# Cyan4973/FiniteStateEntropy

Measured on NVIDIA H100. Metric: encode+decode GB/s (uncompressed) per GPU on 32 KB blocks; bit-exact vs ref, higher is better.
Workload: dtype u8

## Files before the change

### finitestateentropy_b200/csrc/huf_encode.cu

```cuda
#include <cstdlib>
#include <mutex>
#include <vector>
#include "common.cuh"
#include "launch_util.cuh"
#include "fse_dev.cuh"
#include "sink_dev.cuh"
#include "huf_build_dev.cuh"

namespace fseb {
namespace hufe {

constexpr unsigned FULL = 0xFFFFFFFFu;

struct __align__(16) Plan {
    u32 ctable[256];
    u8  header[136];
    u32 hSize;
    u32 state;
    u32 total;
    u32 streamOff[4];
    u32 streamBytes[4];
    u16 segCount[4][256];
};

constexpr int PLAN_WARPS = 8;
constexpr u32 GROUP = 32;
constexpr u32 HDR_STRIDE = 34 + 224 + 1;
constexpr u32 CT_ROW = HDR_STRIDE;
constexpr u32 ROWS = CT_ROW + 256;
constexpr u32 NODE_END = 0x7FFFFFFFu, LEAF_END = 0xFFFFFFFFu;
struct PlanCta {
    u32 nd[ROWS][GROUP];
    u8  sym[256][GROUP];
    u64 res[GROUP];
    u16 msv[GROUP];
    u8  last[GROUP];
    u8  tlog[GROUP];
    u8  live[GROUP];
};
static_assert(ROWS >= 1 + 256 + PLAN_WARPS * 4 * 256 / GROUP, "segment histograms must fit in the rows above the leaves");
static_assert(ROWS >= 1 + 511 && CT_ROW >= 1 + 256, "node rows");
static_assert(HUF_BLOCK_MAX < (1u << 24), "node counts share a word with an 8-bit parent / length");
static_assert(sizeof(PlanCta) <= 76 * 1024, "three CTAs per SM");

__device__ __forceinline__ void warp_hist_range(u32* cnt, const u8* s, u32 begin, u32 end, unsigned lane)
{
    u32 i = begin;
    u32 const head = min(end, (u32)((begin + 15) & ~15u));
    bool const vec = ((reinterpret_cast<u64>(s) & 15) == 0);
    if (vec) {
        for (u32 k = i + lane; k < head; k += 32) atomicAdd(&cnt[s[k]], 1u);
        i = head;
        u32 const nvec = (end - i) / 16;
        const uint4* const gv = reinterpret_cast<const uint4*>(s + i);
        for (u32 v0 = 0; v0 < nvec; v0 += 128) {
            uint4 x[4];
            #pragma unroll
            for (int h = 0; h < 4; h++) { u32 const vi = v0 + 32 * h + lane; x[h] = (vi < nvec) ? __ldg(gv + vi) : make_uint4(0, 0, 0, 0); }
            #pragma unroll
            for (int h = 0; h < 4; h++) {
                if (v0 + 32 * h + lane >= nvec) continue;
                u32 const wd[4] = { x[h].x, x[h].y, x[h].z, x[h].w };
                #pragma unroll
                for (int k = 0; k < 4; k++) {
                    u32 const y = wd[k];
                    atomicAdd(&cnt[y & 0xFF], 1u); atomicAdd(&cnt[__byte_perm(y, 0, 0x4441)], 1u);
                    atomicAdd(&cnt[__byte_perm(y, 0, 0x4442)], 1u); atomicAdd(&cnt[y >> 24], 1u);
                }
            }
        }
        i += nvec * 16;
    }
    for (u32 k = i + lane; k < end; k += 32) atomicAdd(&cnt[s[k]], 1u);
}

__device__ __forceinline__ void warp_hist4_pipelined(u32 (*count4)[256], const u8* s, u32 n, u32 seg, unsigned lane)
{
    const uint4* const gv = reinterpret_cast<const uint4*>(s) + lane;
    u32 const B = n / 2048, perSeg = seg / 2048;
    auto load = [&](uint4 (&x)[4], u32 b) {
        #pragma unroll
        for (int h = 0; h < 4; h++) x[h] = __ldg(gv + b * 128 + 32 * h);
    };
    auto count = [&](const uint4 (&x)[4], u32 b) {
        u32* const cnt = count4[b / perSeg];
        #pragma unroll
        for (int h = 0; h < 4; h++) {
            u32 const wd[4] = { x[h].x, x[h].y, x[h].z, x[h].w };
            #pragma unroll
            for (int k = 0; k < 4; k++) {
                u32 const y = wd[k];
                atomicAdd(&cnt[y & 0xFF], 1u); atomicAdd(&cnt[__byte_perm(y, 0, 0x4441)], 1u);
                atomicAdd(&cnt[__byte_perm(y, 0, 0x4442)], 1u); atomicAdd(&cnt[y >> 24], 1u);
            }
        }
    };
    uint4 xa[4], xb[4];
    load(xa, 0);
    #pragma unroll 1
    for (u32 b = 0; b < B; b += 2) {
        if (b + 1 < B) load(xb, b + 1);
        count(xa, b);
        if (b + 2 < B) load(xa, b + 2);
        if (b + 1 < B) count(xb, b + 1);
    }
}

template <class Geo, int NS>
__global__ void __launch_bounds__(32 * PLAN_WARPS, 3)
huf_plan_kernel(Geo g, u8* __restrict__ cbuf, u64* __restrict__ csizes, const u8* __restrict__ src,
                unsigned msvReq, unsigned tlogReq, Plan* __restrict__ plans)
{
    static_assert(NS == 4 || NS == 1, "4X or 1X");
    extern __shared__ __align__(16) unsigned char smem_raw[];
    PlanCta& S = *reinterpret_cast<PlanCta*>(smem_raw);
    unsigned const lane = threadIdx.x & 31u, warp = threadIdx.x >> 5;
    u32 const b0 = blockIdx.x * GROUP;
#define FSEB_FINAL(v) { if (lane == 0) { P.state = 1; enc_out(g, csizes, b) = (v); S.live[c] = 0; } continue; }

    u32 (*const count4)[256] = reinterpret_cast<u32 (*)[256]>(&S.nd[257][0] + warp * 4 * 256);
    #pragma unroll 1
    for (u32 c = warp; c < GROUP; c += PLAN_WARPS) {
        __syncwarp();
        u32 const b = b0 + c;
        if (b >= g.nBlocks) { if (lane == 0) S.live[c] = 0; continue; }
        u32 const n = enc_len(g, b);
        u64 const cap = enc_cap(g, b);
        const u8* const s = enc_src(g, src, b);
        Plan& P = plans[b];
        if (!n) FSEB_FINAL(0);
        if (!cap) FSEB_FINAL(0);
        if (n > HUF_BLOCK_MAX) FSEB_FINAL(err(E_SRC_WRONG));
        if (tlogReq > HUF_MAX_TLOG) FSEB_FINAL(err(E_TLOG_TOO_LARGE));
        if (msvReq > HUF_MAX_SV) FSEB_FINAL(err(E_MSV_TOO_LARGE));
        unsigned const msvDecl = msvReq ? msvReq : HUF_MAX_SV;

        u32 const seg = (n + 3) / 4;
        for (u32 i = lane; i < 4 * 256; i += 32) (&count4[0][0])[i] = 0;
        __syncwarp();
        if ((reinterpret_cast<u64>(s) & 15) == 0 && seg % 2048 == 0 && n == 4 * seg) warp_hist4_pipelined(count4, s, n, seg, lane);
        else {
            #pragma unroll 1
            for (u32 k = 0; k < 4; k++) {
                u32 const beg = min(k * seg, n), end = (k < 3) ? min((k + 1) * seg, n) : n;
                warp_hist_range(count4[k], s, beg, end, lane);
            }
        }
        __syncwarp();
        u32 cnt[8], top = 0, best = 0;
        #pragma unroll
        for (u32 i = 0; i < 8; i++) {
            u32 const sy = i * 32 + lane;
            cnt[i] = count4[0][sy] + count4[1][sy] + count4[2][sy] + count4[3][sy];
            if (cnt[i]) top = sy;
            best = max(best, cnt[i]);
        }
        #pragma unroll
        for (int dlt = 16; dlt; dlt >>= 1) { top = max(top, __shfl_xor_sync(FULL, top, dlt)); best = max(best, __shfl_xor_sync(FULL, best, dlt)); }
        if (msvDecl < 255 && top > msvDecl) FSEB_FINAL(err(E_MSV_TOO_SMALL));
        if (best == n) { if (lane == 0) enc_dst(g, cbuf, b)[0] = s[0]; FSEB_FINAL(1); }
        if (best <= (n >> 7) + 4) FSEB_FINAL(0);
        u32 const msv = top;
        #pragma unroll
        for (u32 k = 0; k < 4; k++)
            #pragma unroll
            for (u32 i = 0; i < 8; i++) P.segCount[k][i * 32 + lane] = (u16)count4[k][i * 32 + lane];
        u32 key[8], nnz = 0;
        #pragma unroll
        for (u32 i = 0; i < 8; i++) { u32 const sy = i * 32 + lane; key[i] = ((sy <= msv ? cnt[i] : 0u) << 8) | (255u - sy); nnz += __popc(__ballot_sync(FULL, cnt[i] != 0)); }
        warp_sort256_desc(key, lane);
        #pragma unroll
        for (u32 i = 0; i < 8; i++) {
            u32 const r = i * 32 + lane;
            if (r <= msv) { S.nd[1 + r][c] = key[i] >> 8; S.sym[r][c] = (u8)(255u - (key[i] & 0xFFu)); }
        }
        if (lane == 0) {
            S.nd[0][c] = 0;
            S.msv[c] = (u16)msv; S.last[c] = (u8)(nnz - 1); S.live[c] = 1;
            S.tlog[c] = (u8)d_optimal_tablelog(tlogReq ? tlogReq : HUF_DEF_TLOG, n, msv, 1);
        }
    }
    __syncthreads();

    if (warp == 0) {
        u32 const c = lane;
        bool const live = S.live[c];
        u32 const msv = S.msv[c];
        u32* const col = &S.nd[1][c];
        auto at = [&](int i) -> u32& { return col[i * (int)GROUP]; };
        u32* const ct = &S.nd[CT_ROW][c];
        u64 res = 0;
        if (live) {
            int const last = S.last[c];
            int fresh = 256, leaf = last, inner = fresh;
            int const root = fresh + leaf - 1;
            {   u32 const x = at(leaf), y = at(leaf - 1);
                at(fresh) = x + y;
                fresh++; leaf -= 2;
            }
            u32 cl = leaf >= 0 ? at(leaf) : LEAF_END, ci = at(inner);
            while (fresh <= root) {
                int a, bb; u32 ca, cb;
                if (cl < ci) { a = leaf--; ca = cl; cl = leaf >= 0 ? at(leaf) : LEAF_END; } else { a = inner++; ca = ci; ci = inner < fresh ? at(inner) : NODE_END; }
                if (cl < ci) { bb = leaf--; cb = cl; cl = leaf >= 0 ? at(leaf) : LEAF_END; } else { bb = inner++; cb = ci; ci = inner < fresh ? at(inner) : NODE_END; }
                u32 const sum = ca + cb;
                at(fresh) = sum;
                if (inner == fresh) ci = sum;
                u32 const tag = (u32)(fresh - 256) << 24;
                at(a) = ca | tag; at(bb) = cb | tag;
                fresh++;
            }
            at(root) &= 0xFFFFFFu;
            for (int m = root - 1; m >= 256; m--) { u32 const v = at(m); at(m) = (v & 0xFFFFFFu) | (((at(256 + (int)(v >> 24)) >> 24) + 1) << 24); }
            for (int m = 0; m <= last; m++) { u32 const v = at(m); at(m) = (v & 0xFFFFFFu) | (((at(256 + (int)(v >> 24)) >> 24) + 1) << 24); }
            u32 const mb = d_huf_limit_depth(PackedNodeView{ col, (int)GROUP }, (u32)last, S.tlog[c]);
            if (mb > HUF_MAX_TLOG) res = err(E_GENERIC);
            else {
                u32 perLen[HUF_MAX_TLOG + 1], nextVal[HUF_MAX_TLOG + 1];
                for (u32 i = 0; i <= HUF_MAX_TLOG; i++) { perLen[i] = 0; nextVal[i] = 0; }
                for (int m = 0; m <= last; m++) perLen[at(m) >> 24]++;
                u32 v = 0;
                for (int m = (int)mb; m > 0; m--) { nextVal[m] = v; v = (v + perLen[m]) >> 1; }
                for (u32 r = 0; r <= msv; r++) ct[S.sym[r][c] * GROUP] = (int)r <= last ? at((int)r) >> 24 : 0u;
                for (u32 sy = 0; sy <= msv; sy++) { u32 const len = ct[sy * GROUP]; ct[sy * GROUP] = (nextVal[len]++ & 0xFFFF) | (len << 16); }
                S.tlog[c] = (u8)mb;
            }
        }
        __syncwarp();
        if (live && !is_err(res)) {
            u64 const cap = enc_cap(g, b0 + c);
            u32* const area = &S.nd[0][0] + c * HDR_STRIDE;
            struct Col { const u32* p; __device__ u32 operator[](u32 i) const { return p[i * GROUP]; } };
            res = d_huf_write_ctable(reinterpret_cast<u8*>(area), cap < 136 ? cap : 136, Col{ ct }, msv, S.tlog[c], area + 34);
        }
        S.res[c] = res;
    }
    __syncthreads();

    #pragma unroll 1
    for (u32 c = warp; c < GROUP; c += PLAN_WARPS) {
        if (!S.live[c]) continue;
        u32 const b = b0 + c;
        u32 const n = enc_len(g, b);
        u64 const cap = enc_cap(g, b);
        Plan& P = plans[b];
        u64 const hs = S.res[c];
        if (is_err(hs)) FSEB_FINAL(hs);
        if (hs + 12 >= n) FSEB_FINAL(0);
        u64 const capLeft = cap - hs;
        if (NS == 4 && (capLeft < 6 + 1 + 1 + 1 + 8 || n < 12)) FSEB_FINAL(0);
        u32 const msv = S.msv[c];
        u32 cell[8];
        #pragma unroll
        for (u32 i = 0; i < 8; i++) cell[i] = (i * 32 + lane <= msv) ? S.nd[CT_ROW + i * 32 + lane][c] : 0u;
        u32 bits[NS];
        #pragma unroll
        for (int k = 0; k < NS; k++) {
            u32 acc = 0;
            #pragma unroll
            for (u32 i = 0; i < 8; i++) {
                u32 const sy = i * 32 + lane;
                u32 const cnt = (NS == 4) ? (u32)P.segCount[k][sy]
                                          : (u32)P.segCount[0][sy] + P.segCount[1][sy] + P.segCount[2][sy] + P.segCount[3][sy];
                acc += cnt * (cell[i] >> 16);
            }
            #pragma unroll
            for (int dlt = 16; dlt; dlt >>= 1) acc += __shfl_xor_sync(FULL, acc, dlt);
            bits[k] = acc;
        }
        u64 op = (NS == 4) ? 6 : 0; bool fits = true;
        u32 offs[NS], lens[NS];
        #pragma unroll
        for (int t = 0; t < NS; t++) {
            u64 const capk = capLeft - op;
            u64 const tot = (u64)bits[t] + 1;
            if (fits && (capk <= 8 || (tot >> 3) >= capk - 8)) fits = false;
            offs[t] = (u32)(hs + op); lens[t] = (u32)((tot + 7) >> 3);
            op += lens[t];
        }
        u64 const total = hs + op;
        if (!fits || total >= (u64)n - 1) FSEB_FINAL(0);
        #pragma unroll
        for (u32 i = 0; i < 8; i++) P.ctable[i * 32 + lane] = cell[i];
        const u8* const hdr = reinterpret_cast<const u8*>(&S.nd[0][0] + c * HDR_STRIDE);
        for (u32 i = lane; i < (u32)hs; i += 32) P.header[i] = hdr[i];
        if (lane < NS) { P.streamOff[lane] = offs[lane]; P.streamBytes[lane] = lens[lane]; }
        if (lane == 0) { P.hSize = (u32)hs; P.state = 0; P.total = (u32)total; enc_out(g, csizes, b) = total; }
    }
#undef FSEB_FINAL
}

constexpr int THREADS = 128;

template <class Geo>
static __device__ __noinline__ void store_piece_exact(u32* gw, u32 j, uint4 v, u32 a0, u32 endByte)
{
    u32 const wd[4] = { v.x, v.y, v.z, v.w };
    u8* const pb = reinterpret_cast<u8*>(gw + j);
    for (u32 t = 0; t < 16; t++) { u32 const at = 4 * j + t; if (at >= a0 && at < endByte) pb[t] = (u8)(wd[t >> 2] >> (8 * (t & 3))); }
}

template <class Geo, int NS>
__global__ void __launch_bounds__(32 * NS)
huf_emit_kernel(Geo g, u8* __restrict__ cbuf, const u8* __restrict__ src, const Plan* __restrict__ plans, const u32* __restrict__ sharedCT)
{
    static_assert(NS == 4 || NS == 1, "4X or 1X");
    constexpr int NT = 32 * NS;
    constexpr u32 W = 512;
    __shared__ u32 ctab[256];
    constexpr u32 WP = W + 4;
    __shared__ __align__(16) u32 winAll[NS * WP];
    int const tid = threadIdx.x;
    unsigned const lane = tid & 31u; int const k = tid >> 5;
    u32 const b = blockIdx.x;
    const Plan& P = plans[b];
    if (P.state != 0) return;
    u32 const n = enc_len(g, b);
    const u8* const s = enc_src(g, src, b);
    u8* const d = enc_dst(g, cbuf, b);
    u32 const hSize = P.hSize, total = P.total;

    {   const u32* const ct = sharedCT ? sharedCT : P.ctable;
        if constexpr (NS == 4) {
            u32 const c0 = ct[tid], c1 = ct[tid + 128];
            ctab[tid] = (c0 >> 16) | (c0 << 8 & 0xFFFF00u); ctab[tid + 128] = (c1 >> 16) | (c1 << 8 & 0xFFFF00u);
        } else {
            #pragma unroll
            for (int i = tid; i < 256; i += NT) { u32 const c0 = ct[i]; ctab[i] = (c0 >> 16) | (c0 << 8 & 0xFFFF00u); }
        }
    }
    for (u32 i = tid; i < NS * WP; i += NT) winAll[i] = 0;
    for (u32 i = tid; i < hSize; i += NT) d[i] = P.header[i];
    if (NS == 4 && tid < 3) { u32 const v = P.streamBytes[tid]; d[hSize + 2 * tid] = (u8)v; d[hSize + 2 * tid + 1] = (u8)(v >> 8); }
    __syncthreads();
    {
        u32 const seg = (NS == 4) ? (n + 3) / 4 : n;
        int const segBeg = (int)(k * seg);
        int const segEnd = (k < NS - 1) ? (int)((k + 1) * seg) : (int)n;
        u32 sTab = (u32)__cvta_generic_to_shared(ctab);
        asm volatile("mov.u32 %0, %0;" : "+r"(sTab));
        u32* const win = winAll + k * WP;
        u32 sWin = (u32)__cvta_generic_to_shared(win);
        asm volatile("mov.u32 %0, %0;" : "+r"(sWin));
        u8* const gstart = d + P.streamOff[k];
        u32 const a0 = (u32)(reinterpret_cast<u64>(gstart) & 15);
        u32* const gw = reinterpret_cast<u32*>(gstart - a0);
        u32 const sBytes = (k < NS - 1) ? P.streamBytes[k] : total - P.streamOff[NS - 1];
        u32 const endByte = a0 + sBytes;
        u32 bitpos = 8u * a0;
        u32 flushed = 0;
        auto lds32 = [&](u32 a) -> u32 { u32 v; asm volatile("ld.shared.u32 %0, [%1];" : "=r"(v) : "r"(a)); return v; };
        auto lds64 = [&](u32 o) -> uint2 { u32 const e = lds32(sTab + (o >> 1)); return make_uint2(e >> 8, e & 0xFFu); };
        auto red_or = [&](u32 a, u32 v) { asm volatile("red.shared.or.b32 [%0], %1;" :: "r"(a), "r"(v) : "memory"); };
        auto red_or3 = [&](u32 a, u32 v0, u32 v1, u32 v2) {
            asm volatile("red.shared.or.b32 [%0], %1; red.shared.or.b32 [%0+4], %2; red.shared.or.b32 [%0+8], %3;" :: "r"(a), "r"(v0), "r"(v1), "r"(v2) : "memory");
        };
        auto scan = [&](u32 held, u32& excl) -> u32 {
            u32 incl = held;
            #pragma unroll
            for (int dd = 1; dd < 32; dd <<= 1)
                asm volatile("{ .reg .pred p; .reg .u32 t; shfl.sync.up.b32 t|p, %0, %1, 0, 0xffffffff; @p add.u32 %0, %0, t; }" : "+r"(incl) : "r"(dd));
            excl = incl - held;
            return __shfl_sync(FULL, incl, 31);
        };
        auto put = [&](u32 at, u32 x0, u32 x1) {
            u32 const sh = at & 31;
            red_or3(sWin + ((at >> 3) & (4 * (W - 1))), x0 << sh, __funnelshift_l(x0, x1, sh), __funnelshift_l(x1, 0, sh));
        };
        auto put96 = [&](u32 at, u32 z0, u32 z1, u32 z2) {
            u32 const sh = at & 31;
            asm volatile("red.shared.or.b32 [%0], %1; red.shared.or.b32 [%0+4], %2; red.shared.or.b32 [%0+8], %3; red.shared.or.b32 [%0+12], %4;"
                         :: "r"(sWin + ((at >> 3) & (4 * (W - 1)))), "r"(z0 << sh), "r"(__funnelshift_l(z0, z1, sh)), "r"(__funnelshift_l(z1, z2, sh)),
                            "r"(__funnelshift_l(z2, 0, sh)) : "memory");
        };
        auto flush = [&](bool all) {
            u32 const upTo = all ? (endByte + 3) / 4 : (bitpos >> 5);
            if (!all && flushed + 128 > upTo) return;
            __syncwarp();
            while (all ? flushed < upTo : flushed + 128 <= upTo) {
                u32 const j = flushed + 4 * lane;
                if (j < upTo) {
                    u32 const i = j & (W - 1);
                    uint4 v = *reinterpret_cast<uint4*>(win + i);
                    *reinterpret_cast<uint4*>(win + i) = make_uint4(0, 0, 0, 0);
                    if (i == 0) { v.x |= win[W]; v.y |= win[W + 1]; v.z |= win[W + 2]; win[W] = 0; win[W + 1] = 0; win[W + 2] = 0; }
                    if (!all && (j != 0 || a0 == 0)) *reinterpret_cast<uint4*>(gw + j) = v;
                    else store_piece_exact<Geo>(gw, j, v, a0, endByte);
                }
                flushed += 128;
            }
        };
        auto place = [&](u32 x0, u32 x1, u32 held) -> u32 {
            u32 excl; u32 const sum = scan(held, excl);
            put(bitpos + excl, x0, x1);
            return sum;
        };
        constexpr int PF = 4;
        int hiCur = segEnd;
        {
            bool const al8 = ((reinterpret_cast<u64>(s) + (u64)segEnd) & 7) == 0;
            int const nBig = al8 ? (segEnd - segBeg) / 256 : 0;
            const uint2* gq = reinterpret_cast<const uint2*>(s + segEnd) - 1 - lane;
            auto half = [&](u32 w, u32& a0, u32& a1) -> u32 {
                u32 const e0 = lds32(sTab + 4 * __byte_perm(w, 0, 0x4443)), e1 = lds32(sTab + 4 * __byte_perm(w, 0, 0x4442));
                u32 const e2 = lds32(sTab + 4 * __byte_perm(w, 0, 0x4441)), e3 = lds32(sTab + 4 * __byte_perm(w, 0, 0x4440));
                u32 const p01 = (e0 >> 8) | __funnelshift_l(0, e1 >> 8, e0), l01 = e0 + e1;
                u32 const p23 = (e2 >> 8) | __funnelshift_l(0, e3 >> 8, e2), l23 = e2 + e3;
                a0 = p01 | __funnelshift_l(0, p23, l01); a1 = __funnelshift_l(p23, 0, l01);
                return (l01 + l23) & 0xFFu;
            };
            auto merge = [&](u32 x0, u32 x1, u32 lx, u32 y0, u32 y1, u32& z0, u32& z1, u32& z2) {
                u32 const t0 = __funnelshift_l(0, y0, lx), t1 = __funnelshift_l(y0, y1, lx), t2 = __funnelshift_l(y1, 0, lx);
                bool const far = (lx & 32u) != 0;
                z0 = x0 | (far ? 0u : t0); z1 = x1 | (far ? t0 : t1); z2 = far ? t1 : t2;
            };
            auto big2 = [&](uint2 curA, uint2 curB) {
                u32 x0, x1, y0, y1, za0, za1, za2, zb0, zb1, zb2;
                u32 lx = half(curA.y, x0, x1), ly = half(curA.x, y0, y1);
                merge(x0, x1, lx, y0, y1, za0, za1, za2);
                u32 const la = lx + ly;
                lx = half(curB.y, x0, x1); ly = half(curB.x, y0, y1);
                merge(x0, x1, lx, y0, y1, zb0, zb1, zb2);
                u32 const lb = lx + ly;
                u32 excl; u32 const sum = scan(la | (lb << 16), excl);
                u32 const sumA = sum & 0xFFFFu;
                put96(bitpos + (excl & 0xFFFFu), za0, za1, za2);
                put96(bitpos + sumA + (excl >> 16), zb0, zb1, zb2);
                bitpos += sumA + (sum >> 16);
                flush(false);
            };
            constexpr int PB = 2;
            int const rounds = nBig / PB;
            uint2 bufA[PB], bufB[PB];
            #pragma unroll
            for (int i = 0; i < PB; i++) { bufA[i] = rounds > 0 ? __ldg(gq - 32 * i) : make_uint2(0, 0); bufB[i] = make_uint2(0, 0); }
            auto round = [&](uint2 (&X)[PB], uint2 (&Y)[PB], int r) {
                gq -= 32 * PB;
                uint2 const c0 = X[0], c1 = X[1];
                if (r + 1 < rounds) { Y[0] = __ldg(gq); Y[1] = __ldg(gq - 32); }
                big2(c0, c1);
            };
            int r = 0;
            #pragma unroll 1
            for (; r + 1 < rounds; r += 2) { round(bufA, bufB, r); round(bufB, bufA, r + 1); }
            if (r < rounds) round(bufA, bufB, r);
            hiCur -= 256 * rounds * PB;
        }
        bool const wordAligned = ((reinterpret_cast<u64>(s) + (u64)hiCur) & 3) == 0;
        int const nFull = wordAligned ? (hiCur - segBeg) / 128 : 0;
        {
            const u32* gp = reinterpret_cast<const u32*>(s + hiCur) - 1 - lane;
            auto group = [&](u32 o0, u32 o1, u32 o2, u32 o3) {
                uint2 const e0 = lds64(o0), e1 = lds64(o1), e2 = lds64(o2), e3 = lds64(o3);
                u32 const p01 = e0.x | (e1.x << e0.y), l01 = e0.y + e1.y;
                u32 const p23 = e2.x | (e3.x << e2.y), l23 = e2.y + e3.y;
                u32 const a0 = p01 | (p23 << l01), a1 = __funnelshift_l(p23, 0, l01);
                bitpos += place(a0, a1, l01 + l23);
                flush(false);
            };
            int const rounds = nFull / PF;
            u32 bufA[PF], bufB[PF];
            #pragma unroll
            for (int i = 0; i < PF; i++) { bufA[i] = rounds > 0 ? __ldg(gp - 32 * i) : 0u; bufB[i] = 0u; }
            auto round = [&](u32 (&X)[PF], u32 (&Y)[PF], int r) {
                gp -= 32 * PF;
                bool const more = r + 1 < rounds;
                #pragma unroll
                for (int i = 0; i < PF; i++) {
                    u32 const cur = X[i];
                    if (more) Y[i] = __ldg(gp - 32 * i);
                    group(8 * (cur >> 24), 8 * __byte_perm(cur, 0, 0x4442), 8 * __byte_perm(cur, 0, 0x4441), 8 * (cur & 0xFFu));
                }
            };
            int r = 0;
            #pragma unroll 1
            for (; r + 1 < rounds; r += 2) { round(bufA, bufB, r); round(bufB, bufA, r + 1); }
            if (r < rounds) round(bufA, bufB, r);
            for (int j = rounds * PF; j < nFull; j++) {
                u32 const cur = __ldg(reinterpret_cast<const u32*>(s + hiCur) - 1 - lane - 32 * j);
                group(8 * (cur >> 24), 8 * __byte_perm(cur, 0, 0x4442), 8 * __byte_perm(cur, 0, 0x4441), 8 * (cur & 0xFFu));
            }
        }
        {
            int const rest = hiCur - 128 * nFull;
            auto fetch = [&](int hi) -> u32 {
                int const top = hi - 4 * (int)lane;
                u32 v = 0;
                if (top - 4 >= segBeg && ((reinterpret_cast<u64>(s + top) & 3) == 0)) v = __ldg(reinterpret_cast<const u32*>(s + top - 4));
                else if (top > segBeg) {
                    #pragma unroll
                    for (int j = 0; j < 4; j++) { int const i = top - 1 - j; if (i >= segBeg) v |= (u32)s[i] << (8 * (3 - j)); }
                }
                return v;
            };
            #pragma unroll 1
            for (int hi = rest; hi > segBeg; hi -= 128) {
                u32 const cur = fetch(hi);
                int const nValid = hi - 4 * (int)lane - segBeg;
                u64 acc = 0; u32 held = 0;
                #pragma unroll
                for (int j = 0; j < 4; j++) {
                    uint2 const e = lds64(8 * ((cur >> (8 * (3 - j))) & 0xFF));
                    if (j < nValid) { acc |= (u64)e.x << held; held += e.y; }
                }
                bitpos += place((u32)acc, (u32)(acc >> 32), held);
                flush(false);
            }
        }
        if (lane == 0) red_or(sWin + 4 * ((bitpos >> 5) & (W - 1)), 1u << (bitpos & 31));
        bitpos += 1;
        flush(true);
    }
}

__global__ void __launch_bounds__(32 * PLAN_WARPS)
huf_sizes_kernel(BatchGeom g, u64* __restrict__ csizes, const u8* __restrict__ src, const u32* __restrict__ ct, Plan* __restrict__ plans)
{
    __shared__ u8 nbOf[256];
    unsigned const lane = threadIdx.x & 31u;
    for (u32 i = threadIdx.x; i < 256; i += blockDim.x) nbOf[i] = (u8)(ct[i] >> 16);
    __syncthreads();
    u32 const b = blockIdx.x * PLAN_WARPS + (threadIdx.x >> 5);
    if (b >= g.nBlocks) return;
    u32 const n = block_len(g, b);
    const u8* const s = src + (u64)b * g.blockSize;
    u64 const cap = g.slot;
    Plan& P = plans[b];
    if (cap < 6 + 1 + 1 + 1 + 8 || n < 12) { if (lane == 0) { P.state = 1; csizes[b] = 0; } return; }
    u32 const seg = (n + 3) / 4;
    u32 bits[4];
    #pragma unroll 1
    for (u32 k = 0; k < 4; k++) {
        u32 const beg = k * seg, end = (k < 3) ? (k + 1) * seg : n;
        u32 acc = 0;
        u32 i = beg + lane * 4;
        if ((reinterpret_cast<u64>(s + beg) & 3) == 0) {
            for (; i + 4 <= end; i += 128) {
                u32 const w = __ldg(reinterpret_cast<const u32*>(s + i));
                acc += nbOf[w & 0xFF] + nbOf[(w >> 8) & 0xFF] + nbOf[(w >> 16) & 0xFF] + nbOf[w >> 24];
            }
            for (u32 t = i; t < end && t < i + 4; t++) acc += nbOf[s[t]];
        } else for (u32 t = beg + lane; t < end; t += 32) acc += nbOf[s[t]];
        #pragma unroll
        for (int dlt = 16; dlt; dlt >>= 1) acc += __shfl_xor_sync(FULL, acc, dlt);
        bits[k] = acc;
    }
    u64 op = 6; bool fits = true;
    u32 offs[4], lens[4];
    #pragma unroll
    for (int t = 0; t < 4; t++) {
        u64 const capk = cap - op;
        u64 const tot = (u64)bits[t] + 1;
        if (fits && (capk <= 8 || (tot >> 3) >= capk - 8)) fits = false;
        offs[t] = (u32)op; lens[t] = (u32)((tot + 7) >> 3);
        op += lens[t];
    }
    if (!fits) { if (lane == 0) { P.state = 1; csizes[b] = 0; } return; }
    if (lane < 4) { P.streamOff[lane] = offs[lane]; P.streamBytes[lane] = lens[lane]; }
    if (lane == 0) { P.hSize = 0; P.state = 0; P.total = (u32)op; csizes[b] = op; }
}

}

cudaError_t launch_huf_encode_using_ctable(const BatchGeom& g, void* cbuf, u64* csizes, const void* src, const u32* dCTable, cudaStream_t stream)
{
    if (g.nBlocks == 0) return cudaSuccess;
    cudaError_t e;
    hufe::Plan* const plans = (hufe::Plan*)stream_scratch(2, stream, sizeof(hufe::Plan) * (size_t)g.nBlocks, &e);
    if (e != cudaSuccess) return e;
    unsigned const grid = (g.nBlocks + hufe::PLAN_WARPS - 1) / hufe::PLAN_WARPS;
    hufe::huf_sizes_kernel<<<grid, 32 * hufe::PLAN_WARPS, 0, stream>>>(g, csizes, (const u8*)src, dCTable, plans);
    hufe::huf_emit_kernel<BatchGeom, 4><<<g.nBlocks, hufe::THREADS, 0, stream>>>(g, (u8*)cbuf, (const u8*)src, plans, dCTable);
    return cudaGetLastError();
}

namespace {
struct SubBatch { BatchGeom g; u8* cbuf; const u8* src; };
SubBatch sub_batch(const BatchGeom& g, u8* cbuf, const u8* src, u32 b0, u32 n)
{
    BatchGeom gs = g;
    gs.nBlocks = n;
    u64 const off = (u64)b0 * g.blockSize;
    u64 const span = (u64)n * g.blockSize;
    gs.total = (g.total - off < span) ? g.total - off : span;
    return { gs, cbuf + (u64)b0 * g.slot, src + off };
}
struct SubDescs { BlockDescs g; u8* cbuf; const u8* src; };
SubDescs sub_batch(const BlockDescs& g, u8*, const u8*, u32 b0, u32 n) { return { slice(g, b0, n), nullptr, nullptr }; }

template <class Geo, int NS>
cudaError_t huf_encode(const Geo& g, void* cbuf, u64* csizes, const void* src, unsigned msv, unsigned tlog, cudaStream_t stream)
{
    if (g.nBlocks == 0) return cudaSuccess;
    cudaError_t e;
    hufe::Plan* plans = nullptr;
    static int asyncScratch = -1;
    if (asyncScratch < 0) { const char* const v = getenv("FSEB200_SCRATCH_ASYNC"); asyncScratch = (v && atoi(v) == 1) ? 1 : 0; }
    size_t const need = sizeof(hufe::Plan) * (size_t)g.nBlocks;
    if (asyncScratch) e = cudaMallocAsync((void**)&plans, need, stream);
    else plans = (hufe::Plan*)stream_scratch(2, stream, need, &e);
    if (e != cudaSuccess) return e;
    static u32 const subBatch = [] { const char* const v = getenv("FSEB200_HUF_ENC_SUBBATCH"); long n = v ? atol(v) : 0; return (u32)(n < 0 ? 0 : n); }();
    size_t const smem = sizeof(hufe::PlanCta);
    static SmemOptIn optin;
    e = optin.ensure(hufe::huf_plan_kernel<Geo, NS>, current_device(), (int)smem);
    if (e != cudaSuccess) return e;
    u32 const step = (subBatch && subBatch < g.nBlocks) ? subBatch : g.nBlocks;
    for (u32 b0 = 0; b0 < g.nBlocks; b0 += step) {
        auto const sb = sub_batch(g, (u8*)cbuf, (const u8*)src, b0, (g.nBlocks - b0 < step) ? g.nBlocks - b0 : step);
        u64* const cs = csizes ? csizes + b0 : nullptr;
        unsigned const grid = (sb.g.nBlocks + hufe::GROUP - 1) / hufe::GROUP;
        hufe::huf_plan_kernel<Geo, NS><<<grid, 32 * hufe::PLAN_WARPS, smem, stream>>>(sb.g, sb.cbuf, cs, sb.src, msv, tlog, plans + b0);
        hufe::huf_emit_kernel<Geo, NS><<<sb.g.nBlocks, 32 * NS, 0, stream>>>(sb.g, sb.cbuf, sb.src, plans + b0, nullptr);
    }
    e = cudaGetLastError();
    cudaError_t const e2 = asyncScratch ? cudaFreeAsync(plans, stream) : cudaSuccess;
    return e != cudaSuccess ? e : e2;
}
}

cudaError_t launch_huf_encode(const BatchGeom& g, void* cbuf, u64* csizes, const void* src,
                              unsigned msv, unsigned tlog, cudaStream_t stream)
{
    return huf_encode<BatchGeom, 4>(g, cbuf, csizes, src, msv, tlog, stream);
}

cudaError_t launch_huf_encode_blocks(const BlockDescs& g, int nStreams, unsigned msv, unsigned tlog, cudaStream_t stream)
{
    return nStreams == 1 ? huf_encode<BlockDescs, 1>(g, nullptr, nullptr, nullptr, msv, tlog, stream)
                         : huf_encode<BlockDescs, 4>(g, nullptr, nullptr, nullptr, msv, tlog, stream);
}

}
```

Baseline: 399.0.

## Overlap Huffman emit with plan kernel via programmatic dependent launch and ready flags

The plan kernel now triggers launch_dependents at its start and publishes a per-CTA ready flag with a release store after writing its plans. The emit kernel is launched with programmatic stream serialization, and each block spins with acquire loads on its group's flag before reading the plan. The aim is to let emit blocks start as soon as their group's plan is finished instead of waiting for the whole plan grid, hiding the kernel boundary and tail. The cost is an extra memset per sub-batch and spin-waiting emit blocks that occupy SM slots. If plan CTAs are not yet resident while waiting emit blocks fill the SMs, this could contend or even deadlock.

```diff
diff --git a/finitestateentropy_b200/csrc/huf_encode.cu b/finitestateentropy_b200/csrc/huf_encode.cu
--- a/finitestateentropy_b200/csrc/huf_encode.cu
+++ b/finitestateentropy_b200/csrc/huf_encode.cu
@@ -109,9 +109,10 @@
 template <class Geo, int NS>
 __global__ void __launch_bounds__(32 * PLAN_WARPS, 3)
 huf_plan_kernel(Geo g, u8* __restrict__ cbuf, u64* __restrict__ csizes, const u8* __restrict__ src,
-                unsigned msvReq, unsigned tlogReq, Plan* __restrict__ plans)
+                unsigned msvReq, unsigned tlogReq, Plan* __restrict__ plans, u32* __restrict__ ready)
 {
     static_assert(NS == 4 || NS == 1, "4X or 1X");
+    asm volatile("griddepcontrol.launch_dependents;" ::: "memory");
     extern __shared__ __align__(16) unsigned char smem_raw[];
     PlanCta& S = *reinterpret_cast<PlanCta*>(smem_raw);
     unsigned const lane = threadIdx.x & 31u, warp = threadIdx.x >> 5;
@@ -288,6 +289,9 @@
         if (lane == 0) { P.hSize = (u32)hs; P.state = 0; P.total = (u32)total; enc_out(g, csizes, b) = total; }
     }
 #undef FSEB_FINAL
+    __threadfence();
+    __syncthreads();
+    if (threadIdx.x == 0) asm volatile("st.release.gpu.global.u32 [%0], %1;" :: "l"(ready + blockIdx.x), "r"(1u) : "memory");
 }
 
 constexpr int THREADS = 128;
@@ -302,7 +306,8 @@
 
 template <class Geo, int NS>
 __global__ void __launch_bounds__(32 * NS)
-huf_emit_kernel(Geo g, u8* __restrict__ cbuf, const u8* __restrict__ src, const Plan* __restrict__ plans, const u32* __restrict__ sharedCT)
+huf_emit_kernel(Geo g, u8* __restrict__ cbuf, const u8* __restrict__ src, const Plan* plans, const u32* __restrict__ sharedCT,
+                const u32* ready)
 {
     static_assert(NS == 4 || NS == 1, "4X or 1X");
     constexpr int NT = 32 * NS;
@@ -313,6 +318,16 @@
     int const tid = threadIdx.x;
     unsigned const lane = tid & 31u; int const k = tid >> 5;
     u32 const b = blockIdx.x;
+    if (ready) {
+        if (tid == 0)
+            for (;;) {
+                u32 f;
+                asm volatile("ld.acquire.gpu.global.u32 %0, [%1];" : "=r"(f) : "l"(ready + b / GROUP) : "memory");
+                if (f) break;
+                __nanosleep(500);
+            }
+        __syncthreads();
+    }
     const Plan& P = plans[b];
     if (P.state != 0) return;
     u32 const n = enc_len(g, b);
@@ -570,7 +585,7 @@
     if (e != cudaSuccess) return e;
     unsigned const grid = (g.nBlocks + hufe::PLAN_WARPS - 1) / hufe::PLAN_WARPS;
     hufe::huf_sizes_kernel<<<grid, 32 * hufe::PLAN_WARPS, 0, stream>>>(g, csizes, (const u8*)src, dCTable, plans);
-    hufe::huf_emit_kernel<BatchGeom, 4><<<g.nBlocks, hufe::THREADS, 0, stream>>>(g, (u8*)cbuf, (const u8*)src, plans, dCTable);
+    hufe::huf_emit_kernel<BatchGeom, 4><<<g.nBlocks, hufe::THREADS, 0, stream>>>(g, (u8*)cbuf, (const u8*)src, plans, dCTable, nullptr);
     return cudaGetLastError();
 }
 
@@ -596,24 +611,35 @@
     hufe::Plan* plans = nullptr;
     static int asyncScratch = -1;
     if (asyncScratch < 0) { const char* const v = getenv("FSEB200_SCRATCH_ASYNC"); asyncScratch = (v && atoi(v) == 1) ? 1 : 0; }
-    size_t const need = sizeof(hufe::Plan) * (size_t)g.nBlocks;
+    static u32 const subBatch = [] { const char* const v = getenv("FSEB200_HUF_ENC_SUBBATCH"); long n = v ? atol(v) : 0; return (u32)(n < 0 ? 0 : n); }();
+    u32 const step = (subBatch && subBatch < g.nBlocks) ? subBatch : g.nBlocks;
+    u32 const maxGroups = (step + hufe::GROUP - 1) / hufe::GROUP;
+    size_t const need = sizeof(hufe::Plan) * (size_t)g.nBlocks + sizeof(u32) * (size_t)maxGroups;
     if (asyncScratch) e = cudaMallocAsync((void**)&plans, need, stream);
     else plans = (hufe::Plan*)stream_scratch(2, stream, need, &e);
     if (e != cudaSuccess) return e;
-    static u32 const subBatch = [] { const char* const v = getenv("FSEB200_HUF_ENC_SUBBATCH"); long n = v ? atol(v) : 0; return (u32)(n < 0 ? 0 : n); }();
+    u32* const ready = reinterpret_cast<u32*>(plans + g.nBlocks);
     size_t const smem = sizeof(hufe::PlanCta);
     static SmemOptIn optin;
     e = optin.ensure(hufe::huf_plan_kernel<Geo, NS>, current_device(), (int)smem);
     if (e != cudaSuccess) return e;
-    u32 const step = (subBatch && subBatch < g.nBlocks) ? subBatch : g.nBlocks;
-    for (u32 b0 = 0; b0 < g.nBlocks; b0 += step) {
+    cudaLaunchAttribute overlap[1];
+    overlap[0].id = cudaLaunchAttributeProgrammaticStreamSerialization;
+    overlap[0].val.programmaticStreamSerializationAllowed = 1;
+    for (u32 b0 = 0; b0 < g.nBlocks && e == cudaSuccess; b0 += step) {
         auto const sb = sub_batch(g, (u8*)cbuf, (const u8*)src, b0, (g.nBlocks - b0 < step) ? g.nBlocks - b0 : step);
         u64* const cs = csizes ? csizes + b0 : nullptr;
         unsigned const grid = (sb.g.nBlocks + hufe::GROUP - 1) / hufe::GROUP;
-        hufe::huf_plan_kernel<Geo, NS><<<grid, 32 * hufe::PLAN_WARPS, smem, stream>>>(sb.g, sb.cbuf, cs, sb.src, msv, tlog, plans + b0);
-        hufe::huf_emit_kernel<Geo, NS><<<sb.g.nBlocks, 32 * NS, 0, stream>>>(sb.g, sb.cbuf, sb.src, plans + b0, nullptr);
-    }
-    e = cudaGetLastError();
+        e = cudaMemsetAsync(ready, 0, sizeof(u32) * grid, stream);
+        if (e != cudaSuccess) break;
+        hufe::huf_plan_kernel<Geo, NS><<<grid, 32 * hufe::PLAN_WARPS, smem, stream>>>(sb.g, sb.cbuf, cs, sb.src, msv, tlog, plans + b0, ready);
+        cudaLaunchConfig_t cfg = {};
+        cfg.gridDim = dim3(sb.g.nBlocks); cfg.blockDim = dim3(32 * NS); cfg.dynamicSmemBytes = 0; cfg.stream = stream;
+        cfg.attrs = overlap; cfg.numAttrs = 1;
+        e = cudaLaunchKernelEx(&cfg, hufe::huf_emit_kernel<Geo, NS>, sb.g, sb.cbuf, sb.src, (const hufe::Plan*)(plans + b0),
+                               (const u32*)nullptr, (const u32*)ready);
+    }
+    if (e == cudaSuccess) e = cudaGetLastError();
     cudaError_t const e2 = asyncScratch ? cudaFreeAsync(plans, stream) : cudaSuccess;
     return e != cudaSuccess ? e : e2;
 }
```

After: 403.5, median of 6. +1.1%, better.
